# Quantco/tabmat

Measured on AMD Instinct MI355X. Metric: SplitMatrix.sandwich GFLOP/s + effective HBM GB/s, 10M×1k mixed, higher is better.
Workload: dtype f64; 1 GPU; SplitMatrix.sandwich: dense128 + csr512@5% + cats(256,96,32), 10000000 rows/GPU, p=1024, float64 (BASELINE configs[3]); rows_per_gpu=10000000, p=1024, launch=eager, collective=none

## Files before the change

tabmat_amd/csrc/cat.hip:

```cpp
#include <algorithm>

#include "common.hpp"
#include "reduce.hpp"

namespace tmh {

__global__ void fill_i32_kernel(int32_t *p, int64_t n, int32_t v) {
    int64_t i = (int64_t)blockIdx.x * blockDim.x + threadIdx.x;
    if (i < n) p[i] = v;
}

__global__ void scatter_iota_i32_kernel(int32_t *map, const int32_t *cols, int64_t n_cols) {
    int64_t i = (int64_t)blockIdx.x * blockDim.x + threadIdx.x;
    if (i < n_cols) map[cols[i]] = (int32_t)i;
}

int build_col_map(int32_t *map, int64_t m, const int32_t *cols, int64_t n_cols, hipStream_t st) {
    if (m > 0) {
        hipLaunchKernelGGL(fill_i32_kernel, dim3((unsigned)ceil_div(m, 256)), dim3(256), 0, st, map,
                           m, -1);
        TM_LAUNCH_CHECK();
    }
    if (n_cols > 0) {
        hipLaunchKernelGGL(scatter_iota_i32_kernel, dim3((unsigned)ceil_div(n_cols, 256)),
// ... 761 lines not shown
    for (int b = threadIdx.x; b < nel; b += blockDim.x) tile[b] = 0.0;
    __syncthreads();
    const int64_t j0 = (int64_t)blockIdx.y * TJ;
    const int64_t t0 = (int64_t)blockIdx.x * rows_per_block;
    const int64_t t1 = min(t0 + rows_per_block, n);
    for (int64_t k = t0 + threadIdx.x; k < t1; k += blockDim.x) {
        const F dk = d[k];
        int col[MAX_CATS];
#pragma unroll
        for (int c = 0; c < MAX_CATS; ++c)
            col[c] = c < cs.n_cats ? cs.codes[c][k] - cs.drop[c] : -1;
        for (int jl = 0; jl < TJ && j0 + jl < m; ++jl) {
            const F x = dk * M[(j0 + jl) * n + k];
#pragma unroll
            for (int c = 0; c < MAX_CATS; ++c)
                if (col[c] >= 0) atomic_add(&tile[(cs.off[c] + col[c]) * TJ + jl], (lds_acc_t)x);
        }
    }
    __syncthreads();
    F *dst = ws + ((int64_t)blockIdx.y * gridDim.x + blockIdx.x) * stride;
    for (int b = threadIdx.x; b < nel; b += blockDim.x) dst[b] = (F)tile[b];
}

template <typename F>
__global__ void multi_cat_untile_kernel(const F *__restrict__ tmp, int64_t total, int64_t m,
                                        int TJ, F *__restrict__ out) {
    const int64_t e = (int64_t)blockIdx.x * blockDim.x + threadIdx.x;
    if (e >= total * m) return;
    const int64_t a = e / m, j = e % m;
    out[e] = tmp[((j / TJ) * total + a) * TJ + (j % TJ)];
}

template <typename F, bool STAGE>
__global__ __launch_bounds__(1024) void multi_cat_sparse_kernel(
    CatSet cs, const F *__restrict__ d, const F *__restrict__ vals,
    const unsigned *__restrict__ koff, const unsigned char *__restrict__ ecol,
    const int64_t *__restrict__ gptr, int n_groups, int64_t n_slabs, int64_t slabs_per_block,
    int slab_rows, int group_cols, int64_t n, F *__restrict__ ws, int64_t stride) {
    extern __shared__ __attribute__((aligned(16))) unsigned char smem_raw[];
    lds_acc_t *tile = reinterpret_cast<lds_acc_t *>(smem_raw);
    const int tstr = group_cols + 1;
    const int nel = cs.total * tstr;
    for (int b = threadIdx.x; b < nel; b += blockDim.x) tile[b] = 0.0;
    const int g = blockIdx.y;
    const int lane = threadIdx.x & 63;
    const int wave = threadIdx.x >> 6, nwave = blockDim.x >> 6;
    F *sd = reinterpret_cast<F *>(smem_raw + (((size_t)nel * sizeof(lds_acc_t) + 15) / 16) * 16) +
            (size_t)wave * slab_rows;
    int32_t *sc = reinterpret_cast<int32_t *>(
                      reinterpret_cast<F *>(smem_raw + (((size_t)nel * sizeof(lds_acc_t) + 15) / 16) * 16) +
                      (size_t)nwave * slab_rows) +
                  (size_t)wave * cs.n_cats * slab_rows;
    __syncthreads();
    const int64_t s0 = (int64_t)blockIdx.x * slabs_per_block;
    const int64_t s1 = min(s0 + slabs_per_block, n_slabs);
// ... 468 lines not shown
    int rc = make_catset(h_codes, h_ncols, h_drop, n_cats, &cs);
    if (rc) return rc;
    const int64_t total = (int64_t)cs.total * m;
    if (total == 0) return TM_OK;
    if (rows != nullptr) n = n_rows;
    if (n == 0) {
        TM_HIP(hipMemsetAsync(out, 0, sizeof(F) * (size_t)total, st));
        return TM_OK;
    }
    {
        constexpr int VEC = MCW_VEC;
        constexpr int TJW = 16 * VEC;
        const size_t tile_b = ((sizeof(lds_acc_t) * (size_t)cs.total * TJW + 15) / 16) * 16;
        const size_t lds_w = tile_b + (size_t)16 * MCW_RS * (sizeof(F) + (size_t)n_cats * sizeof(int));
        if (!order_f && n_cats <= 8 && m >= VEC && m % VEC == 0 &&
            (reinterpret_cast<uintptr_t>(M) & 15) == 0 && lds_w <= 150 * 1024 &&
            (int64_t)cs.total * TJW * (int64_t)sizeof(lds_acc_t) < (1ll << 30)) {
            const int64_t n_parts = ceil_div(m, TJW);
            const int64_t stride = (int64_t)cs.total * TJW;
            int64_t nblk = std::max<int64_t>(1, tune("catdense_rounds", 1) * NUM_CU / n_parts);
            nblk = std::min<int64_t>(nblk, std::max<int64_t>(1, ceil_div(n, 4096)));
            const int64_t rpb = ceil_div(ceil_div(n, nblk), MCW_RS) * MCW_RS;
            nblk = ceil_div(n, rpb);
            const size_t tmp_bytes = ((sizeof(F) * (size_t)(n_parts * stride) + 255) / 256) * 256;
            void *wsv = nullptr;
            rc = get_workspace(tmp_bytes + sizeof(F) * (size_t)(n_parts * nblk * stride) + 256, &wsv, st);
            if (rc) return rc;
            F *tmp = reinterpret_cast<F *>(wsv);
            F *ws = reinterpret_cast<F *>(reinterpret_cast<char *>(wsv) + tmp_bytes);
            auto gow = [&](auto kern) -> int {
                TM_HIP(hipFuncSetAttribute(reinterpret_cast<const void *>(kern),
                                           hipFuncAttributeMaxDynamicSharedMemorySize, (int)lds_w));
                prof_begin(st);
                const int nw_dflt = (sizeof(F) == 8 && tile_b > 64 * 1024) ? 8 : 16;
                const int nw = (int)std::min<int64_t>(16, std::max<int64_t>(4, tune("catdense_waves", nw_dflt)));
                hipLaunchKernelGGL(kern, dim3((unsigned)nblk, (unsigned)n_parts), dim3(nw * 64), lds_w, st,
                                   cs, d, M, n, m, rpb, ws, stride, rows, wg_log_ptr());
                prof_end(st);
                TM_LAUNCH_CHECK();
                return TM_OK;
            };
            if (n_cats == 1) rc = gow(&multi_cat_dense_wide_kernel<F, 1>);
            else if (n_cats == 2) rc = gow(&multi_cat_dense_wide_kernel<F, 2>);
            else if (n_cats == 3) rc = gow(&multi_cat_dense_wide_kernel<F, 3>);
            else if (n_cats == 4) rc = gow(&multi_cat_dense_wide_kernel<F, 4>);
            else if (n_cats == 5) rc = gow(&multi_cat_dense_wide_kernel<F, 5>);
            else if (n_cats == 6) rc = gow(&multi_cat_dense_wide_kernel<F, 6>);
            else if (n_cats == 7) rc = gow(&multi_cat_dense_wide_kernel<F, 7>);
            else rc = gow(&multi_cat_dense_wide_kernel<F, 8>);
            if (rc) return rc;
            rc = launch_reduce_partials<F>(ws, stride, (int)nblk, (int)n_parts, tmp, n_parts * stride,
                                           false, st);
            if (rc) return rc;
            hipLaunchKernelGGL((multi_cat_untile_kernel<F>), dim3((unsigned)ceil_div(total, 256)),
                               dim3(256), 0, st, tmp, (int64_t)cs.total, m, TJW, out);
            TM_LAUNCH_CHECK();
            return TM_OK;
        }
    }
    if (rows != nullptr) {
        set_error("multi_cat_dense: the row-list form needs the wide-load path");
        return TM_EUNSUPPORTED;
    }
    int TJ = 64;
    while (TJ > 1 && sizeof(lds_acc_t) * (size_t)cs.total * TJ > HIST_LDS_MAX) TJ >>= 1;
    while (TJ > 1 && TJ / 2 >= m) TJ >>= 1;
    if (sizeof(lds_acc_t) * (size_t)cs.total * TJ > HIST_LDS_MAX) {
        set_error("multi_cat_dense: %d stacked categories exceed the LDS tile", cs.total);
        return TM_EUNSUPPORTED;
    }
    const int64_t n_parts = ceil_div(m, TJ);
    const int64_t stride = (int64_t)cs.total * TJ;
    const size_t lds = sizeof(lds_acc_t) * (size_t)stride;
    int64_t nblk = std::max<int64_t>(1, NUM_CU / n_parts);
    nblk = std::min<int64_t>(nblk, std::max<int64_t>(1, ceil_div(n, 4096)));
    const int64_t rpb = ceil_div(n, nblk);
    nblk = ceil_div(n, rpb);
    const size_t tmp_bytes = ((sizeof(F) * (size_t)(n_parts * stride) + 255) / 256) * 256;
    void *wsv = nullptr;
    rc = get_workspace(tmp_bytes + sizeof(F) * (size_t)(n_parts * nblk * stride) + 256, &wsv, st);
    if (rc) return rc;
    F *tmp = reinterpret_cast<F *>(wsv);
    F *ws = reinterpret_cast<F *>(reinterpret_cast<char *>(wsv) + tmp_bytes);
    auto go = [&](auto kern) -> int {
        if (lds > 48 * 1024)
            TM_HIP(hipFuncSetAttribute(reinterpret_cast<const void *>(kern),
                                       hipFuncAttributeMaxDynamicSharedMemorySize, (int)lds));
        prof_begin(st);
        hipLaunchKernelGGL(kern, dim3((unsigned)nblk, (unsigned)n_parts), dim3(1024), lds, st, cs, d,
                           M, n, m, rpb, ws, stride);
        prof_end(st);
        TM_LAUNCH_CHECK();
        return TM_OK;
    };
#define TM_MCD_CASE(V)                                                                       \
    case V:                                                                                  \
        if (order_f) rc = go(&multi_cat_dense_f_kernel<F, V>);                               \
        else if (n_cats == 1) rc = go(&multi_cat_dense_c_kernel<F, V, 1>);                   \
        else if (n_cats == 2) rc = go(&multi_cat_dense_c_kernel<F, V, 2>);                   \
        else if (n_cats == 3) rc = go(&multi_cat_dense_c_kernel<F, V, 3>);                   \
        else if (n_cats == 4) rc = go(&multi_cat_dense_c_kernel<F, V, 4>);                   \
        else rc = go(&multi_cat_dense_c_kernel<F, V, 0>);                                    \
        break;
    switch (TJ) {
        TM_MCD_CASE(64)
        TM_MCD_CASE(32)
        TM_MCD_CASE(16)
        TM_MCD_CASE(8)
        TM_MCD_CASE(4)
        TM_MCD_CASE(2)
        TM_MCD_CASE(1)
        default:
            rc = TM_EINVAL;
    }
#undef TM_MCD_CASE
    if (rc) return rc;
    rc = launch_reduce_partials<F>(ws, stride, (int)nblk, (int)n_parts, tmp, n_parts * stride, false,
                                   st);
    if (rc) return rc;
    hipLaunchKernelGGL((multi_cat_untile_kernel<F>), dim3((unsigned)ceil_div(total, 256)),
                       dim3(256), 0, st, tmp, (int64_t)cs.total, m, TJ, out);
    TM_LAUNCH_CHECK();
    return TM_OK;
}

template <typename F, typename IX>
static int run_multi_cat_sparse_rows(const void *const *h_codes, const int64_t *h_ncols,
                                     const int32_t *h_drop, int n_cats, const F *cm_data,
                                     const IX *cm_ind, const int32_t *ranges, const int32_t *rows,
                                     int64_t n_sel, int64_t m, const F *d_sel, F *out, hipStream_t st);

template <typename F>
static int run_multi_cat_sparse(const void *const *h_codes, const int64_t *h_ncols,
                                const int32_t *h_drop, int n_cats, int64_t n, const F *d,
                                const F *vals, const unsigned *koff, const unsigned char *ecol,
                                const int64_t *gptr, int64_t m, int slab_rows, int group_cols,
                                F *out, hipStream_t st) {
    CatSet cs;
    int rc = make_catset(h_codes, h_ncols, h_drop, n_cats, &cs);
    if (rc) return rc;
    const int64_t total = (int64_t)cs.total * m;
    if (total == 0) return TM_OK;
    if (n == 0) {
        TM_HIP(hipMemsetAsync(out, 0, sizeof(F) * (size_t)total, st));
        return TM_OK;
    }
    const int64_t stride = (int64_t)cs.total * group_cols;
    const size_t tile_bytes = ((sizeof(lds_acc_t) * (size_t)cs.total * (group_cols + 1) + 15) / 16) * 16;
    if (tile_bytes > HIST_LDS_MAX) {
        set_error("multi_cat_sparse: %d stacked categories exceed the LDS tile", cs.total);
        return TM_EUNSUPPORTED;
    }
    const int nw = (int)std::min<int64_t>(16, std::max<int64_t>(4, tune("catsparse_waves", 16)));
    const size_t stage_bytes = (size_t)nw * slab_rows * (sizeof(F) + sizeof(int32_t) * (size_t)n_cats);
    const bool stage = tile_bytes + stage_bytes <= 150 * 1024;
    const size_t lds = tile_bytes + (stage ? stage_bytes : 0);
    const int n_groups = (int)ceil_div(m, group_cols);
    const int64_t n_slabs = ceil_div(n, slab_rows);
    int64_t nblk = std::max<int64_t>(1, tune("catsparse_rounds", 1) * NUM_CU / n_groups);
    nblk = std::min<int64_t>(nblk, n_slabs);
    const int64_t spb = ceil_div(n_slabs, nblk);
    nblk = ceil_div(n_slabs, spb);
    const size_t tmp_bytes = ((sizeof(F) * (size_t)(n_groups * stride) + 255) / 256) * 256;
    void *wsv = nullptr;
    rc = get_workspace(tmp_bytes + sizeof(F) * (size_t)((int64_t)n_groups * nblk * stride) + 256,
                       &wsv, st);
    if (rc) return rc;
    F *tmp = reinterpret_cast<F *>(wsv);
    F *ws = reinterpret_cast<F *>(reinterpret_cast<char *>(wsv) + tmp_bytes);
    if (stage && n_cats <= 8 && slab_rows == 128) {
        auto kpf = n_cats == 1   ? &multi_cat_sparse_pf_kernel<F, 1>
                   : n_cats == 2 ? &multi_cat_sparse_pf_kernel<F, 2>
                   : n_cats == 3 ? &multi_cat_sparse_pf_kernel<F, 3>
                   : n_cats == 4 ? &multi_cat_sparse_pf_kernel<F, 4>
                   : n_cats == 5 ? &multi_cat_sparse_pf_kernel<F, 5>
                   : n_cats == 6 ? &multi_cat_sparse_pf_kernel<F, 6>
                   : n_cats == 7 ? &multi_cat_sparse_pf_kernel<F, 7>
                                 : &multi_cat_sparse_pf_kernel<F, 8>;
        if (lds > 48 * 1024)
            TM_HIP(hipFuncSetAttribute(reinterpret_cast<const void *>(kpf),
                                       hipFuncAttributeMaxDynamicSharedMemorySize, (int)lds));
        prof_begin(st);
        hipLaunchKernelGGL(kpf, dim3((unsigned)nblk, (unsigned)n_groups), dim3(nw * 64), lds, st, cs, d,
                           vals, koff, ecol, gptr, n_groups, n_slabs, spb, group_cols, n, ws, stride,
                           wg_log_ptr());
        prof_end(st);
        TM_LAUNCH_CHECK();
    } else {
        auto kern = stage ? &multi_cat_sparse_kernel<F, true> : &multi_cat_sparse_kernel<F, false>;
        if (lds > 48 * 1024)
            TM_HIP(hipFuncSetAttribute(reinterpret_cast<const void *>(kern),
                                       hipFuncAttributeMaxDynamicSharedMemorySize, (int)lds));
        prof_begin(st);
        hipLaunchKernelGGL(kern, dim3((unsigned)nblk, (unsigned)n_groups), dim3(nw * 64), lds, st, cs,
                           d, vals, koff, ecol, gptr, n_groups, n_slabs, spb, slab_rows, group_cols,
                           n, ws, stride);
        prof_end(st);
        TM_LAUNCH_CHECK();
    }
    rc = launch_reduce_partials<F>(ws, stride, (int)nblk, n_groups, tmp,
                                   (int64_t)n_groups * stride, false, st);
    if (rc) return rc;
    hipLaunchKernelGGL((multi_cat_untile_kernel<F>), dim3((unsigned)ceil_div(total, 256)),
                       dim3(256), 0, st, tmp, (int64_t)cs.total, m, group_cols, out);
    TM_LAUNCH_CHECK();
    return TM_OK;
}

__global__ __launch_bounds__(256) void multi_cat_pack_codes_kernel(CatSet cs, int64_t n, unsigned *__restrict__ out) {
    for (int64_t r = (int64_t)blockIdx.x * blockDim.x + threadIdx.x; r < n; r += (int64_t)gridDim.x * blockDim.x) {
        unsigned pk = 0u;
#pragma unroll
        for (int c = 0; c < 3; ++c) {
            unsigned f = 1023u;
            if (c < cs.n_cats) {
                const int col = cs.codes[c][r] - cs.drop[c];
                if (col >= 0 && col < cs.ncol[c]) f = (unsigned)(cs.off[c] + col);
            }
            pk |= f << (10 * c);
        }
        out[r] = pk;
    }
}

template <typename F>
static int run_multi_cat_sparse_ent(const void *const *h_codes, const int64_t *h_ncols, const int32_t *h_drop,
                                    int n_cats, int64_t n, const F *d, const F *vals, const unsigned short *meta,
                                    const unsigned *bstart, int64_t mk, F *out, hipStream_t st,
                                    const unsigned *packed = nullptr, int64_t n_slots = 0) {
// ... 3 lines not shown
    const int64_t total = (int64_t)cs.total * mk;
    if (total == 0) return TM_OK;
    if (n == 0) {
        TM_HIP(hipMemsetAsync(out, 0, sizeof(F) * (size_t)total, st));
        return TM_OK;
    }
    TM_REQUIRE(mk % 16 == 0 && n_cats >= 1 && n_cats <= 8, "kernel columns in groups of 16, 1 .. 8 categoricals");
    TM_REQUIRE(n < (1ll << 28), "at most 2^28 - 1 rows per block");
    constexpr int GC = 32;
    const int64_t stride = (int64_t)cs.total * GC;
    const size_t lds = ((sizeof(lds_acc_t) * (size_t)cs.total * (GC + 1) + 15) / 16) * 16;
    if (lds > HIST_LDS_MAX) {
        set_error("multi_cat_sparse_ent: %d stacked categories exceed the LDS tile", cs.total);
        return TM_EUNSUPPORTED;
    }
    const int nw = (int)std::min<int64_t>(16, std::max<int64_t>(4, tune("catsparse_waves", 16)));
    const int n_groups = (int)(mk / 16);
    const int n_pairs = (n_groups + 1) / 2;
    const int64_t n_slabs = ceil_div(n, 64);
    int64_t nblk = std::max<int64_t>(1, tune("catsparse_rounds", 1) * NUM_CU / n_pairs);
    nblk = std::min<int64_t>(nblk, n_slabs);
    const int64_t spb = ceil_div(n_slabs, nblk);
    nblk = ceil_div(n_slabs, spb);
    const size_t tmp_bytes = ((sizeof(F) * (size_t)(n_pairs * stride) + 255) / 256) * 256;
    void *wsv = nullptr;
    rc = get_workspace(tmp_bytes + sizeof(F) * (size_t)((int64_t)n_pairs * nblk * stride) + 256, &wsv, st);
    if (rc) return rc;
    F *tmp = reinterpret_cast<F *>(wsv);
    F *ws = reinterpret_cast<F *>(reinterpret_cast<char *>(wsv) + tmp_bytes);
    auto kern = n_cats == 1   ? &multi_cat_sparse_ent_kernel<F, 1>
                : n_cats == 2 ? &multi_cat_sparse_ent_kernel<F, 2>
                : n_cats == 3 ? &multi_cat_sparse_ent_kernel<F, 3>
                : n_cats == 4 ? &multi_cat_sparse_ent_kernel<F, 4>
                : n_cats == 5 ? &multi_cat_sparse_ent_kernel<F, 5>
                : n_cats == 6 ? &multi_cat_sparse_ent_kernel<F, 6>
                : n_cats == 7 ? &multi_cat_sparse_ent_kernel<F, 7>
                              : &multi_cat_sparse_ent_kernel<F, 8>;
    TM_REQUIRE(packed == nullptr || (n_cats <= 3 && cs.total < 1023), "packed codes: at most 3 categoricals, 1022 levels");
    const int ncw = packed != nullptr ? 1 : n_cats;
    const size_t lds_staged = lds + (size_t)nw * 64 * (sizeof(F) + 4 * (size_t)ncw);
    const double fill = (double)n_slots / ((double)std::max(n_groups, 1) * (double)n_slabs);
    if (tune("catsparse_staged", 1) != 0 && lds_staged <= 156 * 1024 &&
        fill >= (double)tune("catsparse_staged_fill", 44)) {
        using KS = void (*)(CatSet, const F *, const F *, const unsigned short *, const unsigned *, int, int64_t, int64_t,
                            int64_t, F *, int64_t, const unsigned *, int);
        KS ks = nullptr;
        if (packed != nullptr) {
            ks = n_cats == 1 ? &multi_cat_sparse_ent_staged_kernel<F, 1, true>
                 : n_cats == 2 ? &multi_cat_sparse_ent_staged_kernel<F, 2, true>
                               : &multi_cat_sparse_ent_staged_kernel<F, 3, true>;
        } else {
            ks = n_cats == 1   ? &multi_cat_sparse_ent_staged_kernel<F, 1, false>
// ... 3 lines not shown
                 : n_cats == 5 ? &multi_cat_sparse_ent_staged_kernel<F, 5, false>
                 : n_cats == 6 ? &multi_cat_sparse_ent_staged_kernel<F, 6, false>
                 : n_cats == 7 ? &multi_cat_sparse_ent_staged_kernel<F, 7, false>
                               : &multi_cat_sparse_ent_staged_kernel<F, 8, false>;
        }
        if (lds_staged > 48 * 1024)
            TM_HIP(hipFuncSetAttribute(reinterpret_cast<const void *>(ks),
                                       hipFuncAttributeMaxDynamicSharedMemorySize, (int)lds_staged));
        prof_begin(st);
        hipLaunchKernelGGL(ks, dim3((unsigned)nblk, (unsigned)n_pairs), dim3(nw * 64), lds_staged, st, cs, d, vals,
                           meta, bstart, n_groups, n, n_slabs, spb, ws, stride, packed, (int)lds);
        prof_end(st);
        TM_LAUNCH_CHECK();
    } else {
        if (lds > 48 * 1024)
            TM_HIP(hipFuncSetAttribute(reinterpret_cast<const void *>(kern),
                                       hipFuncAttributeMaxDynamicSharedMemorySize, (int)lds));
        prof_begin(st);
        hipLaunchKernelGGL(kern, dim3((unsigned)nblk, (unsigned)n_pairs), dim3(nw * 64), lds, st, cs, d, vals, meta,
                           bstart, n_groups, n, n_slabs, spb, ws, stride, packed);
        prof_end(st);
        TM_LAUNCH_CHECK();
    }
    rc = launch_reduce_partials<F>(ws, stride, (int)nblk, n_pairs, tmp, (int64_t)n_pairs * stride, false, st);
    if (rc) return rc;
    hipLaunchKernelGGL((multi_cat_untile_kernel<F>), dim3((unsigned)ceil_div(total, 256)), dim3(256), 0, st, tmp,
                       (int64_t)cs.total, mk, GC, out);
    TM_LAUNCH_CHECK();
    return TM_OK;
}

}

using namespace tmh;

#define TM_CHECK_COMMON(nn) \
    TM_REQUIRE((nn) >= 0, "negative size")

extern "C" {

int tm_cat_transpose_matvec_f32(const int32_t *codes, int64_t n, int64_t n_cols, int drop_first,
                                const float *v, const int32_t *rows, int64_t n_rows,
                                const int32_t *cols, int64_t n_cols_sel, float *out, void *stream) {
    TM_CHECK_COMMON(n);
    return run_cat_tmv<float>(codes, n, n_cols, drop_first, v, rows, n_rows, cols, n_cols_sel, out,
                              as_stream(stream));
}
int tm_cat_transpose_matvec_f64(const int32_t *codes, int64_t n, int64_t n_cols, int drop_first,
                                const double *v, const int32_t *rows, int64_t n_rows,
                                const int32_t *cols, int64_t n_cols_sel, double *out,
                                void *stream) {
    TM_CHECK_COMMON(n);
// ... 218 lines not shown
                                     const IX *cm_ind, const int32_t *ranges, const int32_t *rows,
                                     int64_t n_sel, int64_t m, const F *d_sel, F *out, hipStream_t st) {
    CatSet cs;
    int rc = make_catset(h_codes, h_ncols, h_drop, n_cats, &cs);
    if (rc) return rc;
    const int64_t total = (int64_t)cs.total * m;
    if (total == 0) return TM_OK;
    if (n_sel == 0) {
        TM_HIP(hipMemsetAsync(out, 0, sizeof(F) * (size_t)total, st));
        return TM_OK;
    }
    constexpr int GC = 32;
    const size_t lds = ((sizeof(lds_acc_t) * (size_t)cs.total * (GC + 1) + 15) / 16) * 16;
    if (lds > HIST_LDS_MAX) {
        set_error("multi_cat_sparse_rows: %d stacked categories exceed the LDS tile", cs.total);
        return TM_EUNSUPPORTED;
    }
    const int n_groups = (int)ceil_div(m, GC);
    const int64_t stride = (int64_t)cs.total * GC;
    int64_t nblk = std::max<int64_t>(1, tune("catsparse_rounds", 1) * NUM_CU / n_groups);
    nblk = std::min<int64_t>(nblk, std::max<int64_t>(1, ceil_div(n_sel, 2048)));
    const int64_t rpb = ceil_div(n_sel, nblk);
    nblk = ceil_div(n_sel, rpb);
    const size_t tmp_bytes = ((sizeof(F) * (size_t)(n_groups * stride) + 255) / 256) * 256;
    void *wsv = nullptr;
    rc = get_workspace(tmp_bytes + sizeof(F) * (size_t)((int64_t)n_groups * nblk * stride) + 256, &wsv, st);
    if (rc) return rc;
    F *tmp = reinterpret_cast<F *>(wsv);
    F *ws = reinterpret_cast<F *>(reinterpret_cast<char *>(wsv) + tmp_bytes);
    auto kern = &multi_cat_sparse_rows_kernel<F, IX>;
    if (lds > 48 * 1024)
        TM_HIP(hipFuncSetAttribute(reinterpret_cast<const void *>(kern),
                                   hipFuncAttributeMaxDynamicSharedMemorySize, (int)lds));
    prof_begin(st);
    hipLaunchKernelGGL(kern, dim3((unsigned)nblk, (unsigned)n_groups), dim3(1024), lds, st, cs, cm_data,
                       cm_ind, ranges, rows, d_sel, n_sel, rpb, ws, stride);
    prof_end(st);
    TM_LAUNCH_CHECK();
    rc = launch_reduce_partials<F>(ws, stride, (int)nblk, n_groups, tmp, (int64_t)n_groups * stride, false, st);
    if (rc) return rc;
    hipLaunchKernelGGL((multi_cat_untile_kernel<F>), dim3((unsigned)ceil_div(total, 256)), dim3(256), 0,
                       st, tmp, (int64_t)cs.total, m, GC, out);
    TM_LAUNCH_CHECK();
    return TM_OK;
}
}

extern "C" {
int tm_multi_cat_sparse_sandwich_rows_f32(const void *const *h_codes, const int64_t *h_ncols,
                                          const int32_t *h_drop_first, int n_cats,
                                          const float *cm_data, const int32_t *cm_indices,
                                          const int32_t *row_ranges, const int32_t *rows,
                                          int64_t n_sel, int64_t m, const float *d_sel, float *out,
                                          void *stream) {
    return tmh::run_multi_cat_sparse_rows<float, int32_t>(h_codes, h_ncols, h_drop_first, n_cats, cm_data,
                                                 cm_indices, row_ranges, rows, n_sel, m, d_sel, out,
                                                 tmh::as_stream(stream));
}
int tm_multi_cat_sparse_sandwich_rows_f64(const void *const *h_codes, const int64_t *h_ncols,
                                          const int32_t *h_drop_first, int n_cats,
                                          const double *cm_data, const int32_t *cm_indices,
                                          const int32_t *row_ranges, const int32_t *rows,
                                          int64_t n_sel, int64_t m, const double *d_sel, double *out,
                                          void *stream) {
    return tmh::run_multi_cat_sparse_rows<double, int32_t>(h_codes, h_ncols, h_drop_first, n_cats, cm_data,
                                                  cm_indices, row_ranges, rows, n_sel, m, d_sel, out,
                                                  tmh::as_stream(stream));
// ... 23 lines not shown
```

tabmat_amd/csrc/reduce.hpp:

```cpp
#pragma once
#include "common.hpp"

namespace tmh {

template <typename F, bool ACCUMULATE, int NW>
__global__ __launch_bounds__(NW * 64) void reduce_partials_kernel(const F *__restrict__ ws,
                                                                  int64_t stride, int nb,
                                                                  F *__restrict__ out,
                                                                  int64_t out_elems) {
    __shared__ double red[NW][64];
    const int lane = threadIdx.x & 63;
    const int wave = threadIdx.x >> 6;
    const int64_t e = (int64_t)blockIdx.x * 64 + lane;
    const int part = blockIdx.y;
    double acc = 0.0;
    if (e < stride) {
        const F *p = ws + ((int64_t)part * nb) * stride + e;
        for (int b = wave; b < nb; b += NW) acc += (double)p[(int64_t)b * stride];
    }
    red[wave][lane] = acc;
    __syncthreads();
    if (wave == 0 && e < stride) {
        const int64_t o = (int64_t)part * stride + e;
        if (o < out_elems) {
// ... 12 lines not shown
template <typename F>
inline int launch_reduce_partials(const F *ws, int64_t stride, int nb, int n_parts, F *out,
                                  int64_t out_elems, bool accumulate, hipStream_t st) {
    dim3 grid((unsigned)ceil_div(stride, 64), (unsigned)n_parts);
    const bool small = (int64_t)grid.x * grid.y < 1024 && nb > 16;
    if (small) {
        if (accumulate)
            hipLaunchKernelGGL((reduce_partials_kernel<F, true, 16>), grid, dim3(1024), 0, st, ws,
                               stride, nb, out, out_elems);
        else
            hipLaunchKernelGGL((reduce_partials_kernel<F, false, 16>), grid, dim3(1024), 0, st, ws,
                               stride, nb, out, out_elems);
    } else if (accumulate) {
        hipLaunchKernelGGL((reduce_partials_kernel<F, true, 4>), grid, dim3(256), 0, st, ws, stride,
                           nb, out, out_elems);
    } else {
        hipLaunchKernelGGL((reduce_partials_kernel<F, false, 4>), grid, dim3(256), 0, st, ws, stride,
                           nb, out, out_elems);
    }
    TM_LAUNCH_CHECK();
    return TM_OK;
}

__global__ void fill_i32_kernel(int32_t *p, int64_t n, int32_t v);
__global__ void scatter_iota_i32_kernel(int32_t *map, const int32_t *cols, int64_t n_cols);

int build_col_map(int32_t *map, int64_t m, const int32_t *cols, int64_t n_cols, hipStream_t st);

}
```

tabmat_amd/csrc/sparse_blocks.hip:

```cpp
#include <algorithm>

#include "common.hpp"
#include "reduce.hpp"

namespace tmh {

constexpr int KB_WAVES = 16;
constexpr int KB_TS = 128;

template <typename F>
__global__ void blocks_assemble_kernel(const F *__restrict__ tiles, int n_out, F *__restrict__ out) {
    const int j = blockIdx.x * blockDim.x + threadIdx.x;
    const int i = blockIdx.y;
    if (i >= n_out || j >= n_out) return;
    const int hi = max(i, j), lo = min(i, j);
    const int I = hi / KB_TS, J = lo / KB_TS;
    const int part = I * (I + 1) / 2 + J;
    out[(int64_t)i * n_out + j] = tiles[(int64_t)part * KB_TS * KB_TS + (hi % KB_TS) * KB_TS + (lo % KB_TS)];
}

constexpr int KB_FLAG_REP_A = 1 << 16;
constexpr int KB_FLAG_REP_B = 1 << 17;

template <typename F, bool U8, bool D12 = false>
__global__ __launch_bounds__(KB_WAVES * 64) void sparse_sandwich_blocks_kernel(
    const F *__restrict__ data, const int32_t *__restrict__ ind, const int32_t *__restrict__ cptr,
    int64_t n, int64_t nnz1, const int32_t *__restrict__ blocks, const int4 *__restrict__ wg_tab,
    const F *__restrict__ d, int max_nb, F *__restrict__ ws, WgLogBuf *__restrict__ wglog) {
    constexpr int TS = KB_TS;
    const unsigned long long t_begin = wg_log_begin(wglog);
    extern __shared__ __attribute__((aligned(16))) unsigned char smem_raw[];
    lds_acc_t *tile = reinterpret_cast<lds_acc_t *>(smem_raw);
    const int4 w = wg_tab[2 * blockIdx.x], x = wg_tab[2 * blockIdx.x + 1];
    const int part = __builtin_amdgcn_readfirstlane(w.x), slot = __builtin_amdgcn_readfirstlane(w.y);
    const int b0 = __builtin_amdgcn_readfirstlane(w.z), b1 = __builtin_amdgcn_readfirstlane(w.w);
    const int bfull = __builtin_amdgcn_readfirstlane(x.x);
    int wfull = __builtin_amdgcn_readfirstlane(x.y);
    {
        const int nwv = (int)(blockDim.x >> 6);
        if (nwv != KB_WAVES) {
            wfull = (wfull * nwv + KB_WAVES / 2) / KB_WAVES;
// ... 152 lines not shown
    F *dst = ws + ((int64_t)part * max_nb + slot) * (TS * TS);
    for (int b = threadIdx.x; b < TS * TS; b += blockDim.x) {
        const int r = b / TS, c = b % TS;
        dst[b] = (F)tile[r * TS + (c ^ ((r & 15) << 3))];
    }
}

template <typename F, bool U8 = false, bool D12 = false>
static int run_sparse_sandwich_blocks(const F *data, const int32_t *ind, const int32_t *cptr, int64_t n,
                                      int64_t m, int64_t nnz, const int32_t *blocks, const int32_t *wg_tab,
                                      int n_wg, int max_nb, const F *d, F *out, hipStream_t st) {
    if (m == 0) return TM_OK;
    if (n == 0 || nnz == 0 || n_wg == 0) {
        TM_HIP(hipMemsetAsync(out, 0, sizeof(F) * (size_t)(m * m), st));
        return TM_OK;
    }
    constexpr int TS = KB_TS;
    const int nchunk = (int)ceil_div(m, TS);
    const int n_parts = nchunk * (nchunk + 1) / 2;
    TM_REQUIRE(nnz < (1ll << 31) && n < (1ll << 29), "sparse block too large for the block-list sandwich");
    TM_REQUIRE(!D12 || n < (1ll << 24), "12-byte block descriptors hold 24 bits of row");
    TM_REQUIRE(max_nb >= 1 && n_wg >= 1, "empty workgroup table");
    const size_t lds = sizeof(lds_acc_t) * (size_t)(TS * TS);
    const size_t tmp_bytes = (sizeof(F) * (size_t)n_parts * TS * TS + 255) / 256 * 256;
    const size_t ws_bytes = sizeof(F) * (size_t)n_parts * (size_t)max_nb * TS * TS;
    void *wsv = nullptr;
    int rc = get_workspace(tmp_bytes + ws_bytes + 256, &wsv, st);
    if (rc) return rc;
    F *tmp = reinterpret_cast<F *>(wsv);
    F *ws = reinterpret_cast<F *>(reinterpret_cast<char *>(wsv) + tmp_bytes);
    TM_HIP(hipMemsetAsync(ws, 0, ws_bytes, st));
    auto kern = &sparse_sandwich_blocks_kernel<F, U8, D12>;
    TM_HIP(hipFuncSetAttribute(reinterpret_cast<const void *>(kern),
                               hipFuncAttributeMaxDynamicSharedMemorySize, (int)lds));
    prof_begin(st);
    const int kb_waves = (int)std::min<int64_t>(KB_WAVES, std::max<int64_t>(2, tune("k2b_waves", KB_WAVES)));
    hipLaunchKernelGGL(kern, dim3((unsigned)n_wg), dim3(kb_waves * 64), lds, st, data, ind, cptr, n, nnz - 1,
                       blocks, reinterpret_cast<const int4 *>(wg_tab), d,
                       max_nb, ws, wg_log_ptr());
    prof_end(st);
    TM_LAUNCH_CHECK();
    rc = launch_reduce_partials<F>(ws, (int64_t)TS * TS, max_nb, n_parts, tmp, (int64_t)n_parts * TS * TS,
                                   false, st);
    if (rc) return rc;
    hipLaunchKernelGGL((blocks_assemble_kernel<F>), dim3((unsigned)ceil_div(m, 64), (unsigned)m), dim3(64),
                       0, st, tmp, (int)m, out);
    TM_LAUNCH_CHECK();
    return TM_OK;
}

}

extern "C" {

int tm_sparse_sandwich_blocks_f32(const float *cm_data, const int32_t *cm_indices, const int32_t *cptr,
                                  int64_t n, int64_t m, int64_t nnz, const int32_t *blocks,
                                  const int32_t *wg_tab, int n_wg, int max_nb, const float *d, float *out,
                                  void *stream) {
    return tmh::run_sparse_sandwich_blocks<float>(cm_data, cm_indices, cptr, n, m, nnz, blocks, wg_tab, n_wg,
                                                  max_nb, d, out, tmh::as_stream(stream));
}
int tm_sparse_sandwich_blocks_f64(const double *cm_data, const int32_t *cm_indices, const int32_t *cptr,
                                  int64_t n, int64_t m, int64_t nnz, const int32_t *blocks,
                                  const int32_t *wg_tab, int n_wg, int max_nb, const double *d, double *out,
                                  void *stream) {
    return tmh::run_sparse_sandwich_blocks<double>(cm_data, cm_indices, cptr, n, m, nnz, blocks, wg_tab, n_wg,
                                                   max_nb, d, out, tmh::as_stream(stream));
}

// ... 36 lines not shown
```

tabmat_amd/csrc/sparse_ent.hip:

```cpp
#include "common.hpp"
#include "reduce.hpp"

namespace tmh {

constexpr int EN_R = 64;
constexpr int EN_C = 16;
constexpr int EN_NW = 16;
constexpr int EN_THREADS = EN_NW * 64;
constexpr int EN_W = 128;
constexpr int EN_B = 16;
constexpr int EN_SB = 64;

template <typename F>
struct EnLds {
    static constexpr int ROWB = EN_W * (int)sizeof(F);
    static constexpr int SLABB = EN_R * ROWB;
    static constexpr int SCR_OFF = ROWB + 2 * SLABB;
    static constexpr int CS_OFF = SCR_OFF + EN_NW * EN_SB * 16;
    static constexpr int TOTAL = CS_OFF + EN_NW * EN_C * (int)sizeof(double);
};

constexpr int EN_CVGPR = 24;
#define EN_LD "40"

// ... 296 lines not shown

    if (active) {
        F *dst = ws + (((int64_t)blockIdx.y * gridDim.x + blockIdx.x) * n_groups + group) * (EN_C * EN_W);
        static_for<EN_C>([&](auto jc) {
            constexpr int j = decltype(jc)::value;
            if constexpr (sizeof(F) == 8) {
                const u4 o = u4{en_read_acc<4 * j>(), en_read_acc<4 * j + 1>(), en_read_acc<4 * j + 2>(),
                                en_read_acc<4 * j + 3>()};
                *reinterpret_cast<u4 *>(dst + j * EN_W + 2 * lane) = o;
            } else {
                typedef unsigned u2 __attribute__((ext_vector_type(2)));
                const u2 o = u2{en_read_acc<2 * j>(), en_read_acc<2 * j + 1>()};
                *reinterpret_cast<u2 *>(dst + j * EN_W + 2 * lane) = o;
            }
        });
        if constexpr (CSUM) {
            if (blockIdx.y == 0 && lane < EN_C)
                ws_csum[(int64_t)blockIdx.x * (n_groups * EN_C) + group * EN_C + lane] = (F)cs_lds[lane];
        }
    }
}

template <typename F>
__global__ void en_untile_kernel(const F *__restrict__ tmp, int64_t m, int64_t nB, F *__restrict__ out) {
    const int64_t e = (int64_t)blockIdx.x * blockDim.x + threadIdx.x;
    if (e >= m * nB) return;
    const int64_t i = e / nB, j = e % nB;
    out[e] = tmp[((j / EN_W) * m + i) * EN_W + (j % EN_W)];
}

template <typename F>
__global__ void en_csum_kernel(const F *__restrict__ part, int nblk, int64_t m, F *__restrict__ csum) {
    const int64_t c = (int64_t)blockIdx.x * blockDim.x + threadIdx.x;
    if (c >= m) return;
    double a = 0.0;
    for (int b = 0; b < nblk; ++b) a += (double)part[(int64_t)b * m + c];
    csum[c] = (F)a;
}

template <typename F>
static int run_csr_dense_ent(const F *vals, const uint16_t *meta, const uint32_t *bstart, int64_t n, int64_t m,
                             const F *B, int64_t r, const F *d, F *out, F *colsum, hipStream_t st) {
    const int64_t nB = r;
    const int64_t total = m * nB;
    if (total == 0) return TM_OK;
    constexpr int VEC = 16 / (int)sizeof(F);
    if ((reinterpret_cast<uintptr_t>(B) & 15) != 0 || r % VEC != 0 || nB < VEC) {
        set_error("tm_csr_dense_sandwich_ent: B must be C-ordered with 16-byte aligned rows");
        return TM_EUNSUPPORTED;
    }
    if (m % EN_C != 0) {
        set_error("tm_csr_dense_sandwich_ent: m must be a multiple of tm_ent_group_cols()");
        return TM_EINVAL;
    }
    if (n >= (1ll << 28)) {
        set_error("tm_csr_dense_sandwich_ent: at most 2^28 - 1 rows per block (work in row parts)");
        return TM_EUNSUPPORTED;
    }
    const int64_t n_slabs = ceil_div(n, EN_R);
    const int n_groups = (int)(m / EN_C);
    const int n_parts = (int)ceil_div(nB, EN_W);
    const int nz = (int)ceil_div(n_groups, EN_NW);
    const bool want_csum = colsum != nullptr;
    if (n_slabs == 0) {
        TM_HIP(hipMemsetAsync(out, 0, sizeof(F) * (size_t)total, st));
        if (want_csum) TM_HIP(hipMemsetAsync(colsum, 0, sizeof(F) * (size_t)m, st));
        return TM_OK;
    }
    int64_t nblk = std::max<int64_t>(1, tune("ent_rounds", 1) * NUM_CU / ((int64_t)n_parts * nz));
    nblk = std::min<int64_t>(nblk, n_slabs);
    const int64_t spb = ceil_div(n_slabs, nblk);
    nblk = ceil_div(n_slabs, spb);
    const int64_t stride = m * EN_W;
    const size_t tmp_bytes = (sizeof(F) * (size_t)(n_parts * stride) + 255) / 256 * 256;
    const size_t part_bytes = (sizeof(F) * (size_t)((int64_t)n_parts * nblk * stride) + 255) / 256 * 256;
    const size_t csum_bytes = ((want_csum ? sizeof(F) * (size_t)(nblk * m) : 0) + 255) / 256 * 256 + 256;
    void *wsv = nullptr;
    int rc = get_workspace(tmp_bytes + part_bytes + csum_bytes + 256, &wsv, st);
    if (rc) return rc;
    F *tmp = reinterpret_cast<F *>(wsv);
    F *ws = reinterpret_cast<F *>(reinterpret_cast<char *>(wsv) + tmp_bytes);
    F *ws_csum = reinterpret_cast<F *>(reinterpret_cast<char *>(wsv) + tmp_bytes + part_bytes);
    const size_t lds = (size_t)EnLds<F>::TOTAL;
    auto kern = want_csum ? &csr_dense_ent_kernel<F, true> : &csr_dense_ent_kernel<F, false>;
    TM_HIP(hipFuncSetAttribute(reinterpret_cast<const void *>(kern),
                               hipFuncAttributeMaxDynamicSharedMemorySize, (int)lds));
    prof_begin(st);
    hipLaunchKernelGGL(kern, dim3((unsigned)nblk, (unsigned)n_parts, (unsigned)nz), dim3(EN_THREADS), lds, st,
                       vals, meta, bstart, n_groups, n_slabs, spb, B, n, r, (int)nB, d, ws, ws_csum,
                       reinterpret_cast<long long *>((uintptr_t)tune("ent_prof", 0)));
    prof_end(st);
    TM_LAUNCH_CHECK();
    rc = launch_reduce_partials<F>(ws, stride, (int)nblk, n_parts, tmp, n_parts * stride, false, st);
    if (rc) return rc;
    hipLaunchKernelGGL((en_untile_kernel<F>), dim3((unsigned)ceil_div(total, 256)), dim3(256), 0, st, tmp, m,
                       nB, out);
    TM_LAUNCH_CHECK();
    if (want_csum) {
        hipLaunchKernelGGL((en_csum_kernel<F>), dim3((unsigned)ceil_div(m, 256)), dim3(256), 0, st, ws_csum,
                           (int)nblk, m, colsum);
        TM_LAUNCH_CHECK();
    }
    return TM_OK;
}

}

extern "C" {
int tm_ent_rows(void) { return tmh::EN_R; }
int tm_ent_group_cols(void) { return tmh::EN_C; }
int tm_ent_batch_slots(void) { return tmh::EN_B; }

int tm_csr_dense_sandwich_ent_f32(const float *vals, const uint16_t *meta, const uint32_t *bstart, int64_t n,
                                  int64_t m, const float *B, int64_t r, const float *d, float *out,
                                  float *colsum, void *stream) {
    return tmh::run_csr_dense_ent<float>(vals, meta, bstart, n, m, B, r, d, out, colsum, tmh::as_stream(stream));
}
int tm_csr_dense_sandwich_ent_f64(const double *vals, const uint16_t *meta, const uint32_t *bstart, int64_t n,
                                  int64_t m, const double *B, int64_t r, const double *d, double *out,
                                  double *colsum, void *stream) {
// ... 4 lines not shown
```

Baseline: 1036 GB/s.

## Fuse partial reduction with untile and block assembly in sandwich epilogues

Replaces the separate reduce-partials kernel followed by an untile/assemble kernel with a single kernel that sums per-block partials and writes directly to the final output layout. This applies across the categorical, dense-ent and sparse-block sandwich paths. The sparse-block path also drops the workspace memset and sums only the workgroups listed in the workgroup table, using an LDS bitmap. This removes an intermediate buffer round-trip through HBM and some launches, but the new kernels use scattered output writes and assume unwritten partial slots are never read.

```diff
diff --git a/tabmat_amd/csrc/cat.hip b/tabmat_amd/csrc/cat.hip
--- a/tabmat_amd/csrc/cat.hip
+++ b/tabmat_amd/csrc/cat.hip
@@ -807,15 +807,6 @@
     for (int b = threadIdx.x; b < nel; b += blockDim.x) dst[b] = (F)tile[b];
 }
 
-template <typename F>
-__global__ void multi_cat_untile_kernel(const F *__restrict__ tmp, int64_t total, int64_t m,
-                                        int TJ, F *__restrict__ out) {
-    const int64_t e = (int64_t)blockIdx.x * blockDim.x + threadIdx.x;
-    if (e >= total * m) return;
-    const int64_t a = e / m, j = e % m;
-    out[e] = tmp[((j / TJ) * total + a) * TJ + (j % TJ)];
-}
-
 template <typename F, bool STAGE>
 __global__ __launch_bounds__(1024) void multi_cat_sparse_kernel(
     CatSet cs, const F *__restrict__ d, const F *__restrict__ vals,
@@ -1330,12 +1321,10 @@
             nblk = std::min<int64_t>(nblk, std::max<int64_t>(1, ceil_div(n, 4096)));
             const int64_t rpb = ceil_div(ceil_div(n, nblk), MCW_RS) * MCW_RS;
             nblk = ceil_div(n, rpb);
-            const size_t tmp_bytes = ((sizeof(F) * (size_t)(n_parts * stride) + 255) / 256) * 256;
             void *wsv = nullptr;
-            rc = get_workspace(tmp_bytes + sizeof(F) * (size_t)(n_parts * nblk * stride) + 256, &wsv, st);
+            rc = get_workspace(sizeof(F) * (size_t)(n_parts * nblk * stride) + 256, &wsv, st);
             if (rc) return rc;
-            F *tmp = reinterpret_cast<F *>(wsv);
-            F *ws = reinterpret_cast<F *>(reinterpret_cast<char *>(wsv) + tmp_bytes);
+            F *ws = reinterpret_cast<F *>(wsv);
             auto gow = [&](auto kern) -> int {
                 TM_HIP(hipFuncSetAttribute(reinterpret_cast<const void *>(kern),
                                            hipFuncAttributeMaxDynamicSharedMemorySize, (int)lds_w));
@@ -1357,13 +1346,7 @@
             else if (n_cats == 7) rc = gow(&multi_cat_dense_wide_kernel<F, 7>);
             else rc = gow(&multi_cat_dense_wide_kernel<F, 8>);
             if (rc) return rc;
-            rc = launch_reduce_partials<F>(ws, stride, (int)nblk, (int)n_parts, tmp, n_parts * stride,
-                                           false, st);
-            if (rc) return rc;
-            hipLaunchKernelGGL((multi_cat_untile_kernel<F>), dim3((unsigned)ceil_div(total, 256)),
-                               dim3(256), 0, st, tmp, (int64_t)cs.total, m, TJW, out);
-            TM_LAUNCH_CHECK();
-            return TM_OK;
+            return launch_reduce_partials_untile<F>(ws, (int64_t)cs.total, TJW, (int)nblk, (int)n_parts, m, out, st);
         }
     }
     if (rows != nullptr) {
@@ -1384,12 +1367,10 @@
     nblk = std::min<int64_t>(nblk, std::max<int64_t>(1, ceil_div(n, 4096)));
     const int64_t rpb = ceil_div(n, nblk);
     nblk = ceil_div(n, rpb);
-    const size_t tmp_bytes = ((sizeof(F) * (size_t)(n_parts * stride) + 255) / 256) * 256;
     void *wsv = nullptr;
-    rc = get_workspace(tmp_bytes + sizeof(F) * (size_t)(n_parts * nblk * stride) + 256, &wsv, st);
+    rc = get_workspace(sizeof(F) * (size_t)(n_parts * nblk * stride) + 256, &wsv, st);
     if (rc) return rc;
-    F *tmp = reinterpret_cast<F *>(wsv);
-    F *ws = reinterpret_cast<F *>(reinterpret_cast<char *>(wsv) + tmp_bytes);
+    F *ws = reinterpret_cast<F *>(wsv);
     auto go = [&](auto kern) -> int {
         if (lds > 48 * 1024)
             TM_HIP(hipFuncSetAttribute(reinterpret_cast<const void *>(kern),
@@ -1423,13 +1404,7 @@
     }
 #undef TM_MCD_CASE
     if (rc) return rc;
-    rc = launch_reduce_partials<F>(ws, stride, (int)nblk, (int)n_parts, tmp, n_parts * stride, false,
-                                   st);
-    if (rc) return rc;
-    hipLaunchKernelGGL((multi_cat_untile_kernel<F>), dim3((unsigned)ceil_div(total, 256)),
-                       dim3(256), 0, st, tmp, (int64_t)cs.total, m, TJ, out);
-    TM_LAUNCH_CHECK();
-    return TM_OK;
+    return launch_reduce_partials_untile<F>(ws, (int64_t)cs.total, TJ, (int)nblk, (int)n_parts, m, out, st);
 }
 
 template <typename F, typename IX>
@@ -1469,13 +1444,10 @@
     nblk = std::min<int64_t>(nblk, n_slabs);
     const int64_t spb = ceil_div(n_slabs, nblk);
     nblk = ceil_div(n_slabs, spb);
-    const size_t tmp_bytes = ((sizeof(F) * (size_t)(n_groups * stride) + 255) / 256) * 256;
     void *wsv = nullptr;
-    rc = get_workspace(tmp_bytes + sizeof(F) * (size_t)((int64_t)n_groups * nblk * stride) + 256,
-                       &wsv, st);
+    rc = get_workspace(sizeof(F) * (size_t)((int64_t)n_groups * nblk * stride) + 256, &wsv, st);
     if (rc) return rc;
-    F *tmp = reinterpret_cast<F *>(wsv);
-    F *ws = reinterpret_cast<F *>(reinterpret_cast<char *>(wsv) + tmp_bytes);
+    F *ws = reinterpret_cast<F *>(wsv);
     if (stage && n_cats <= 8 && slab_rows == 128) {
         auto kpf = n_cats == 1   ? &multi_cat_sparse_pf_kernel<F, 1>
                    : n_cats == 2 ? &multi_cat_sparse_pf_kernel<F, 2>
@@ -1506,13 +1478,7 @@
         prof_end(st);
         TM_LAUNCH_CHECK();
     }
-    rc = launch_reduce_partials<F>(ws, stride, (int)nblk, n_groups, tmp,
-                                   (int64_t)n_groups * stride, false, st);
-    if (rc) return rc;
-    hipLaunchKernelGGL((multi_cat_untile_kernel<F>), dim3((unsigned)ceil_div(total, 256)),
-                       dim3(256), 0, st, tmp, (int64_t)cs.total, m, group_cols, out);
-    TM_LAUNCH_CHECK();
-    return TM_OK;
+    return launch_reduce_partials_untile<F>(ws, (int64_t)cs.total, group_cols, (int)nblk, n_groups, m, out, st);
 }
 
 __global__ __launch_bounds__(256) void multi_cat_pack_codes_kernel(CatSet cs, int64_t n, unsigned *__restrict__ out) {
@@ -1562,12 +1528,10 @@
     nblk = std::min<int64_t>(nblk, n_slabs);
     const int64_t spb = ceil_div(n_slabs, nblk);
     nblk = ceil_div(n_slabs, spb);
-    const size_t tmp_bytes = ((sizeof(F) * (size_t)(n_pairs * stride) + 255) / 256) * 256;
     void *wsv = nullptr;
-    rc = get_workspace(tmp_bytes + sizeof(F) * (size_t)((int64_t)n_pairs * nblk * stride) + 256, &wsv, st);
+    rc = get_workspace(sizeof(F) * (size_t)((int64_t)n_pairs * nblk * stride) + 256, &wsv, st);
     if (rc) return rc;
-    F *tmp = reinterpret_cast<F *>(wsv);
-    F *ws = reinterpret_cast<F *>(reinterpret_cast<char *>(wsv) + tmp_bytes);
+    F *ws = reinterpret_cast<F *>(wsv);
     auto kern = n_cats == 1   ? &multi_cat_sparse_ent_kernel<F, 1>
                 : n_cats == 2 ? &multi_cat_sparse_ent_kernel<F, 2>
                 : n_cats == 3 ? &multi_cat_sparse_ent_kernel<F, 3>
@@ -1617,12 +1581,7 @@
         prof_end(st);
         TM_LAUNCH_CHECK();
     }
-    rc = launch_reduce_partials<F>(ws, stride, (int)nblk, n_pairs, tmp, (int64_t)n_pairs * stride, false, st);
-    if (rc) return rc;
-    hipLaunchKernelGGL((multi_cat_untile_kernel<F>), dim3((unsigned)ceil_div(total, 256)), dim3(256), 0, st, tmp,
-                       (int64_t)cs.total, mk, GC, out);
-    TM_LAUNCH_CHECK();
-    return TM_OK;
+    return launch_reduce_partials_untile<F>(ws, (int64_t)cs.total, GC, (int)nblk, n_pairs, mk, out, st);
 }
 
 }
@@ -1887,12 +1846,10 @@
     nblk = std::min<int64_t>(nblk, std::max<int64_t>(1, ceil_div(n_sel, 2048)));
     const int64_t rpb = ceil_div(n_sel, nblk);
     nblk = ceil_div(n_sel, rpb);
-    const size_t tmp_bytes = ((sizeof(F) * (size_t)(n_groups * stride) + 255) / 256) * 256;
     void *wsv = nullptr;
-    rc = get_workspace(tmp_bytes + sizeof(F) * (size_t)((int64_t)n_groups * nblk * stride) + 256, &wsv, st);
+    rc = get_workspace(sizeof(F) * (size_t)((int64_t)n_groups * nblk * stride) + 256, &wsv, st);
     if (rc) return rc;
-    F *tmp = reinterpret_cast<F *>(wsv);
-    F *ws = reinterpret_cast<F *>(reinterpret_cast<char *>(wsv) + tmp_bytes);
+    F *ws = reinterpret_cast<F *>(wsv);
     auto kern = &multi_cat_sparse_rows_kernel<F, IX>;
     if (lds > 48 * 1024)
         TM_HIP(hipFuncSetAttribute(reinterpret_cast<const void *>(kern),
@@ -1902,12 +1859,7 @@
                        cm_ind, ranges, rows, d_sel, n_sel, rpb, ws, stride);
     prof_end(st);
     TM_LAUNCH_CHECK();
-    rc = launch_reduce_partials<F>(ws, stride, (int)nblk, n_groups, tmp, (int64_t)n_groups * stride, false, st);
-    if (rc) return rc;
-    hipLaunchKernelGGL((multi_cat_untile_kernel<F>), dim3((unsigned)ceil_div(total, 256)), dim3(256), 0,
-                       st, tmp, (int64_t)cs.total, m, GC, out);
-    TM_LAUNCH_CHECK();
-    return TM_OK;
+    return launch_reduce_partials_untile<F>(ws, (int64_t)cs.total, GC, (int)nblk, n_groups, m, out, st);
 }
 }
 
diff --git a/tabmat_amd/csrc/reduce.hpp b/tabmat_amd/csrc/reduce.hpp
--- a/tabmat_amd/csrc/reduce.hpp
+++ b/tabmat_amd/csrc/reduce.hpp
@@ -58,6 +58,50 @@
     return TM_OK;
 }
 
+template <typename F, int NW>
+__global__ __launch_bounds__(NW * 64) void reduce_partials_untile_kernel(const F *__restrict__ ws,
+                                                                         int64_t stride, int nb, int TJ,
+                                                                         int64_t m, F *__restrict__ out) {
+    __shared__ double red[NW][64];
+    const int lane = threadIdx.x & 63;
+    const int wave = threadIdx.x >> 6;
+    const int64_t e = (int64_t)blockIdx.x * 64 + lane;
+    const int part = blockIdx.y;
+    double acc = 0.0;
+    if (e < stride) {
+        const F *p = ws + ((int64_t)part * nb) * stride + e;
+        for (int b = wave; b < nb; b += NW) acc += (double)p[(int64_t)b * stride];
+    }
+    red[wave][lane] = acc;
+    __syncthreads();
+    if (wave == 0 && e < stride) {
+        const int64_t a = e / TJ, j = (int64_t)part * TJ + e % TJ;
+        if (j < m) {
+            double s = 0.0;
+#pragma unroll
+            for (int w = 0; w < NW; w += 4)
+                s += (red[w][lane] + red[w + 1][lane]) + (red[w + 2][lane] + red[w + 3][lane]);
+            out[a * m + j] = (F)s;
+        }
+    }
+}
+
+template <typename F>
+inline int launch_reduce_partials_untile(const F *ws, int64_t rows, int TJ, int nb, int n_parts, int64_t m,
+                                         F *out, hipStream_t st) {
+    const int64_t stride = rows * TJ;
+    dim3 grid((unsigned)ceil_div(stride, 64), (unsigned)n_parts);
+    const bool small = (int64_t)grid.x * grid.y < 1024 && nb > 16;
+    if (small)
+        hipLaunchKernelGGL((reduce_partials_untile_kernel<F, 16>), grid, dim3(1024), 0, st, ws, stride, nb, TJ,
+                           m, out);
+    else
+        hipLaunchKernelGGL((reduce_partials_untile_kernel<F, 4>), grid, dim3(256), 0, st, ws, stride, nb, TJ, m,
+                           out);
+    TM_LAUNCH_CHECK();
+    return TM_OK;
+}
+
 __global__ void fill_i32_kernel(int32_t *p, int64_t n, int32_t v);
 __global__ void scatter_iota_i32_kernel(int32_t *map, const int32_t *cols, int64_t n_cols);
 
diff --git a/tabmat_amd/csrc/sparse_blocks.hip b/tabmat_amd/csrc/sparse_blocks.hip
--- a/tabmat_amd/csrc/sparse_blocks.hip
+++ b/tabmat_amd/csrc/sparse_blocks.hip
@@ -8,15 +8,83 @@
 constexpr int KB_WAVES = 16;
 constexpr int KB_TS = 128;
 
-template <typename F>
-__global__ void blocks_assemble_kernel(const F *__restrict__ tiles, int n_out, F *__restrict__ out) {
-    const int j = blockIdx.x * blockDim.x + threadIdx.x;
-    const int i = blockIdx.y;
-    if (i >= n_out || j >= n_out) return;
-    const int hi = max(i, j), lo = min(i, j);
-    const int I = hi / KB_TS, J = lo / KB_TS;
-    const int part = I * (I + 1) / 2 + J;
-    out[(int64_t)i * n_out + j] = tiles[(int64_t)part * KB_TS * KB_TS + (hi % KB_TS) * KB_TS + (lo % KB_TS)];
+constexpr int KB_FIN_G = 2;
+constexpr int KB_MAX_NB = 1 << 12;
+
+template <typename F, int NW>
+__global__ __launch_bounds__(NW * 64) void blocks_finish_kernel(const F *__restrict__ ws,
+                                                                const int4 *__restrict__ wg_tab, int n_wg,
+                                                                int max_nb, int n_out, F *__restrict__ out) {
+    constexpr int TS = KB_TS;
+    constexpr int G = KB_FIN_G;
+    extern __shared__ __attribute__((aligned(16))) unsigned char fin_raw[];
+    __shared__ double red[G][NW][64];
+    __shared__ int cnt[NW];
+    const int per = (max_nb + NW - 1) / NW;
+    int *list = reinterpret_cast<int *>(fin_raw);
+    unsigned *bits = reinterpret_cast<unsigned *>(list + NW * per);
+    const int nword = (max_nb + 31) >> 5;
+    const int part = blockIdx.y;
+    for (int k = threadIdx.x; k < nword; k += blockDim.x) bits[k] = 0u;
+    __syncthreads();
+    for (int k = threadIdx.x; k < n_wg; k += blockDim.x) {
+        const int2 ps = *reinterpret_cast<const int2 *>(wg_tab + 2 * (int64_t)k);
+        if (ps.x == part && (unsigned)ps.y < (unsigned)max_nb) atomicOr(&bits[ps.y >> 5], 1u << (ps.y & 31));
+    }
+    __syncthreads();
+    if (threadIdx.x < NW) {
+        int c = 0;
+        for (int b = threadIdx.x; b < max_nb; b += NW)
+            if ((bits[b >> 5] >> (b & 31)) & 1u) list[threadIdx.x * per + c++] = b;
+        cnt[threadIdx.x] = c;
+    }
+    __syncthreads();
+    const int lane = threadIdx.x & 63;
+    const int wave = threadIdx.x >> 6;
+    const int e0 = blockIdx.x * (G * 64) + lane;
+    const F *p = ws + (int64_t)part * max_nb * (TS * TS) + e0;
+    const int *mine = list + wave * per;
+    const int nmine = cnt[wave];
+    double acc[G];
+#pragma unroll
+    for (int g = 0; g < G; ++g) acc[g] = 0.0;
+    int k = 0;
+    for (; k + 4 <= nmine; k += 4) {
+        F v[4][G];
+#pragma unroll
+        for (int u = 0; u < 4; ++u)
+#pragma unroll
+            for (int g = 0; g < G; ++g) v[u][g] = p[(int64_t)mine[k + u] * (TS * TS) + 64 * g];
+#pragma unroll
+        for (int u = 0; u < 4; ++u)
+#pragma unroll
+            for (int g = 0; g < G; ++g) acc[g] += (double)v[u][g];
+    }
+    for (; k < nmine; ++k)
+#pragma unroll
+        for (int g = 0; g < G; ++g) acc[g] += (double)p[(int64_t)mine[k] * (TS * TS) + 64 * g];
+#pragma unroll
+    for (int g = 0; g < G; ++g) red[g][wave][lane] = acc[g];
+    __syncthreads();
+    if (wave != 0) return;
+    int I = (int)((sqrtf(8.0f * (float)part + 1.0f) - 1.0f) * 0.5f);
+    while ((I + 1) * (I + 2) / 2 <= part) ++I;
+    while (I * (I + 1) / 2 > part) --I;
+    const int J = part - I * (I + 1) / 2;
+#pragma unroll
+    for (int g = 0; g < G; ++g) {
+        double s = 0.0;
+#pragma unroll
+        for (int w = 0; w < NW; w += 4)
+            s += (red[g][w][lane] + red[g][w + 1][lane]) + (red[g][w + 2][lane] + red[g][w + 3][lane]);
+        const int e = e0 + 64 * g;
+        const int r = e / TS, c = e % TS;
+        const int i = I * TS + r, j = J * TS + c;
+        if (i < n_out && j < n_out && (I != J || c <= r)) {
+            out[(int64_t)i * n_out + j] = (F)s;
+            if (i != j) out[(int64_t)j * n_out + i] = (F)s;
+        }
+    }
 }
 
 constexpr int KB_FLAG_REP_A = 1 << 16;
@@ -215,14 +283,12 @@
     TM_REQUIRE(!D12 || n < (1ll << 24), "12-byte block descriptors hold 24 bits of row");
     TM_REQUIRE(max_nb >= 1 && n_wg >= 1, "empty workgroup table");
     const size_t lds = sizeof(lds_acc_t) * (size_t)(TS * TS);
-    const size_t tmp_bytes = (sizeof(F) * (size_t)n_parts * TS * TS + 255) / 256 * 256;
+    TM_REQUIRE(max_nb <= KB_MAX_NB, "too many workgroups per tile for the block-list sandwich");
     const size_t ws_bytes = sizeof(F) * (size_t)n_parts * (size_t)max_nb * TS * TS;
     void *wsv = nullptr;
-    int rc = get_workspace(tmp_bytes + ws_bytes + 256, &wsv, st);
+    int rc = get_workspace(ws_bytes + 256, &wsv, st);
     if (rc) return rc;
-    F *tmp = reinterpret_cast<F *>(wsv);
-    F *ws = reinterpret_cast<F *>(reinterpret_cast<char *>(wsv) + tmp_bytes);
-    TM_HIP(hipMemsetAsync(ws, 0, ws_bytes, st));
+    F *ws = reinterpret_cast<F *>(wsv);
     auto kern = &sparse_sandwich_blocks_kernel<F, U8, D12>;
     TM_HIP(hipFuncSetAttribute(reinterpret_cast<const void *>(kern),
                                hipFuncAttributeMaxDynamicSharedMemorySize, (int)lds));
@@ -233,11 +299,16 @@
                        max_nb, ws, wg_log_ptr());
     prof_end(st);
     TM_LAUNCH_CHECK();
-    rc = launch_reduce_partials<F>(ws, (int64_t)TS * TS, max_nb, n_parts, tmp, (int64_t)n_parts * TS * TS,
-                                   false, st);
-    if (rc) return rc;
-    hipLaunchKernelGGL((blocks_assemble_kernel<F>), dim3((unsigned)ceil_div(m, 64), (unsigned)m), dim3(64),
-                       0, st, tmp, (int)m, out);
+    const dim3 fgrid((unsigned)(TS * TS / (64 * KB_FIN_G)), (unsigned)n_parts);
+    const bool small = (int64_t)(TS * TS / 64) * n_parts < 1024 && max_nb > 16;
+    const int nw = small ? 16 : 4;
+    const size_t flds = sizeof(int) * (size_t)(nw * ceil_div(max_nb, nw)) + sizeof(unsigned) * (size_t)ceil_div(max_nb, 32);
+    if (small)
+        hipLaunchKernelGGL((blocks_finish_kernel<F, 16>), fgrid, dim3(1024), flds, st, ws,
+                           reinterpret_cast<const int4 *>(wg_tab), n_wg, max_nb, (int)m, out);
+    else
+        hipLaunchKernelGGL((blocks_finish_kernel<F, 4>), fgrid, dim3(256), flds, st, ws,
+                           reinterpret_cast<const int4 *>(wg_tab), n_wg, max_nb, (int)m, out);
     TM_LAUNCH_CHECK();
     return TM_OK;
 }
diff --git a/tabmat_amd/csrc/sparse_ent.hip b/tabmat_amd/csrc/sparse_ent.hip
--- a/tabmat_amd/csrc/sparse_ent.hip
+++ b/tabmat_amd/csrc/sparse_ent.hip
@@ -342,14 +342,6 @@
 }
 
 template <typename F>
-__global__ void en_untile_kernel(const F *__restrict__ tmp, int64_t m, int64_t nB, F *__restrict__ out) {
-    const int64_t e = (int64_t)blockIdx.x * blockDim.x + threadIdx.x;
-    if (e >= m * nB) return;
-    const int64_t i = e / nB, j = e % nB;
-    out[e] = tmp[((j / EN_W) * m + i) * EN_W + (j % EN_W)];
-}
-
-template <typename F>
 __global__ void en_csum_kernel(const F *__restrict__ part, int nblk, int64_t m, F *__restrict__ csum) {
     const int64_t c = (int64_t)blockIdx.x * blockDim.x + threadIdx.x;
     if (c >= m) return;
@@ -392,15 +384,13 @@
     const int64_t spb = ceil_div(n_slabs, nblk);
     nblk = ceil_div(n_slabs, spb);
     const int64_t stride = m * EN_W;
-    const size_t tmp_bytes = (sizeof(F) * (size_t)(n_parts * stride) + 255) / 256 * 256;
     const size_t part_bytes = (sizeof(F) * (size_t)((int64_t)n_parts * nblk * stride) + 255) / 256 * 256;
     const size_t csum_bytes = ((want_csum ? sizeof(F) * (size_t)(nblk * m) : 0) + 255) / 256 * 256 + 256;
     void *wsv = nullptr;
-    int rc = get_workspace(tmp_bytes + part_bytes + csum_bytes + 256, &wsv, st);
+    int rc = get_workspace(part_bytes + csum_bytes + 256, &wsv, st);
     if (rc) return rc;
-    F *tmp = reinterpret_cast<F *>(wsv);
-    F *ws = reinterpret_cast<F *>(reinterpret_cast<char *>(wsv) + tmp_bytes);
-    F *ws_csum = reinterpret_cast<F *>(reinterpret_cast<char *>(wsv) + tmp_bytes + part_bytes);
+    F *ws = reinterpret_cast<F *>(wsv);
+    F *ws_csum = reinterpret_cast<F *>(reinterpret_cast<char *>(wsv) + part_bytes);
     const size_t lds = (size_t)EnLds<F>::TOTAL;
     auto kern = want_csum ? &csr_dense_ent_kernel<F, true> : &csr_dense_ent_kernel<F, false>;
     TM_HIP(hipFuncSetAttribute(reinterpret_cast<const void *>(kern),
@@ -411,11 +401,8 @@
                        reinterpret_cast<long long *>((uintptr_t)tune("ent_prof", 0)));
     prof_end(st);
     TM_LAUNCH_CHECK();
-    rc = launch_reduce_partials<F>(ws, stride, (int)nblk, n_parts, tmp, n_parts * stride, false, st);
+    rc = launch_reduce_partials_untile<F>(ws, m, EN_W, (int)nblk, n_parts, nB, out, st);
     if (rc) return rc;
-    hipLaunchKernelGGL((en_untile_kernel<F>), dim3((unsigned)ceil_div(total, 256)), dim3(256), 0, st, tmp, m,
-                       nB, out);
-    TM_LAUNCH_CHECK();
     if (want_csum) {
         hipLaunchKernelGGL((en_csum_kernel<F>), dim3((unsigned)ceil_div(m, 256)), dim3(256), 0, st, ws_csum,
                            (int)nblk, m, colsum);
```

Result: no change. 1042 GB/s (median of 4 runs) (+0.5%).
